# bibymaths/phoskintime

Measured on AMD Instinct MI355X. Metric: ODE-solve replicas/sec (32-state distributive, 14 tp), higher is better.
Workload: dtype f64

## Files before the change

phoskintime_amd/csrc/pk_dist_fast.hpp:

```cpp
#pragma once
#include "pk_dist_rows.hpp"
#include "pk_env.hpp"

namespace pk {

template <int G, int RPL>
__device__ __forceinline__ double site_sum(const double (&s)[RPL], int lane) { return gsum<G>(tree_sum(s), lane); }

enum { PK_DM_NONE = 0, PK_DM_SUM = 1, PK_DM_FULL = 2 };
__host__ __device__ __forceinline__ int dist_metric_class(const SolveArgs& A) {
  return !A.metric ? PK_DM_NONE : (A.metric_id == PK_METRIC_TOTAL_SIGNAL || A.metric_id == PK_METRIC_MEAN_ACTIVITY) ? PK_DM_SUM : PK_DM_FULL;
}
template <bool CLIP, bool NORM, bool FLAT, bool SOL, int MC>
struct DistFixed {
  static constexpr int SLOT_MC = MC;
  static constexpr bool LITERAL = false;
  __host__ __device__ static __forceinline__ bool clip(const SolveArgs&) { return CLIP; }
  __host__ __device__ static __forceinline__ bool normalize(const SolveArgs&) { return NORM; }
  __host__ __device__ static __forceinline__ bool flat(const SolveArgs&) { return FLAT; }
  __host__ __device__ static __forceinline__ bool sol(const SolveArgs&) { return SOL; }
  __host__ __device__ static __forceinline__ int mclass(const SolveArgs&) { return MC; }
  static bool matches(const SolveArgs& A) {
    return (A.clip != 0) == CLIP && (A.normalize != 0) == NORM && (A.flat != nullptr) == FLAT && (A.sol != nullptr) == SOL && dist_metric_class(A) == MC;
  }
};
struct DistAny {
  static constexpr int SLOT_MC = PK_DM_FULL;
  static constexpr bool LITERAL = true;
  __host__ __device__ static __forceinline__ bool clip(const SolveArgs& A) { return A.clip != 0; }
  __host__ __device__ static __forceinline__ bool normalize(const SolveArgs& A) { return A.normalize != 0; }
  __host__ __device__ static __forceinline__ bool flat(const SolveArgs& A) { return A.flat != nullptr; }
  __host__ __device__ static __forceinline__ bool sol(const SolveArgs& A) { return A.sol != nullptr; }
  __host__ __device__ static __forceinline__ int mclass(const SolveArgs& A) { return dist_metric_class(A); }
  static bool matches(const SolveArgs&) { return true; }
};
using DistSolSum = DistFixed<true, false, false, true, PK_DM_SUM>;
using DistSolOnly = DistFixed<true, false, false, true, PK_DM_NONE>;
using DistFlatOnly = DistFixed<true, false, true, false, PK_DM_NONE>;

template <int RPL, int MC, bool RES = false> constexpr int dist_fast_slots() {
  return MC == PK_DM_FULL ? 3 * RPL + (RES ? 4 : 6) : MC == PK_DM_SUM ? 2 * RPL + 1 : 2 * RPL;
}

template <int RPL, bool PARK, int NT> struct Parked;
template <int RPL, int NT> struct Parked<RPL, false, NT> {
  double v[3 * RPL + 6];
  __device__ __forceinline__ explicit Parked(double*) {}
  template <int K> __device__ __forceinline__ double get() const { return v[K]; }
  template <int K> __device__ __forceinline__ void set(double x) { v[K] = x; }
  __device__ __forceinline__ void fence() {}
};
template <int RPL, int NT> struct Parked<RPL, true, NT> {
  typedef __attribute__((address_space(3))) double lds_double;
  lds_double* base;
  __device__ __forceinline__ explicit Parked(double* lds) : base((lds_double*)lds + threadIdx.x) {}
  template <int K> __device__ __forceinline__ double get() const { return base[K * NT]; }
  template <int K> __device__ __forceinline__ void set(double x) { base[K * NT] = x; }
  __device__ __forceinline__ void fence() { asm volatile("" : "+v"(base)); }
};
template <int RPL, bool PARK, int NT = 256, class CFG = DistAny, bool RES = false>
constexpr size_t dist_fast_lds_bytes() { return PARK ? (size_t)(dist_fast_slots<RPL, CFG::SLOT_MC, RES>() + RPL) * NT * sizeof(double) : 0; }

constexpr int PK_DSCHED_K2 = 5, PK_DSCHED_K1 = 9;
constexpr int PK_HWREG_HW_ID = 4 | (31 << 11), PK_HWREG_HW_ID_WAVE = 4 | (3 << 11), PK_HWREG_XCC_ID = 20 | (31 << 11);

template <bool PACE> struct DistPace {
  __device__ __forceinline__ void enter(const SolveArgs&) {}
  __device__ __forceinline__ void step(int) const {}
};
template <> struct DistPace<true> {
  bool paced = false;
  __device__ __forceinline__ void enter(const SolveArgs& A) {
    const int sched = A.sched;
    if (sched != PK_DSCHED_OFF) {
      bool leader = false;
      if ((int)gridDim.x > A.R1) {
        if (sched & PK_DSCHED_LEAD_SLOT) leader = (int)blockIdx.x < A.R1 && __builtin_amdgcn_s_getreg(PK_HWREG_HW_ID_WAVE) == 0;
        if (sched & PK_DSCHED_LEAD_BLOCK) leader = leader || (int)blockIdx.x < A.R1 / 3;
      }
      if (leader) __builtin_amdgcn_s_setprio(3);
      paced = !leader && (sched & PK_DSCHED_LEVEL) != 0;
    }
  }
  __device__ __forceinline__ void step(const int k) const {
    if (paced) {
      if (__builtin_amdgcn_ballot_w64(k < PK_DSCHED_K2) != 0) __builtin_amdgcn_s_setprio(2);
      else if (__builtin_amdgcn_ballot_w64(k < PK_DSCHED_K1) != 0) __builtin_amdgcn_s_setprio(1);
      else __builtin_amdgcn_s_setprio(0);
    }
  }
};

struct DistTraceRec {
  unsigned long long t_entry, t_exit;
  unsigned block, hw_id, xcc_id, iters;
};
struct DistTraceBuf { DistTraceRec* rec; long long capacity; };
template <int TRACE> struct DistTrace;

template <int TRACE> struct DistWaveTrace {
  int witer = 0;
  __device__ __forceinline__ void enter() {
    const unsigned long long t0 = __builtin_amdgcn_s_memrealtime();
    const DistTraceBuf tb = DistTrace<TRACE>::get();
    if (threadIdx.x == 0 && tb.rec && (long long)blockIdx.x < tb.capacity) {
      DistTraceRec* r = tb.rec + blockIdx.x;
      r->t_entry = t0; r->t_exit = 0; r->block = blockIdx.x; r->iters = 0;
      r->hw_id = __builtin_amdgcn_s_getreg(PK_HWREG_HW_ID); r->xcc_id = __builtin_amdgcn_s_getreg(PK_HWREG_XCC_ID);
    }
  }
  __device__ __forceinline__ void step() { ++witer; }
  __device__ __forceinline__ void exit() const {
    int it = witer;
    for (int o = 32; o > 0; o >>= 1) { const int v = __shfl_xor(it, o); it = v > it ? v : it; }
    const DistTraceBuf tb = DistTrace<TRACE>::get();
    if (threadIdx.x == 0 && tb.rec && (long long)blockIdx.x < tb.capacity) {
      DistTraceRec* r = tb.rec + blockIdx.x;
      r->iters = (unsigned)it; r->t_exit = __builtin_amdgcn_s_memrealtime();
    }
  }
};
template <> struct DistWaveTrace<0> {
  __device__ __forceinline__ void enter() {}
  __device__ __forceinline__ void step() {}
  __device__ __forceinline__ void exit() const {}
};

template <int METHOD, int RPL, bool PARK, bool RES> constexpr bool dist_scaled() {
  return PARK && ResolventTab<METHOD>::DIFFERENCE && (RES ? (RPL == 6 || RPL == 8) : (RPL >= 5 && RPL <= 7));
}
constexpr double PK_DIST_SCALE_MIN = 0x1p-600;

template <int G, int RPL, int METHOD, bool PARK = false, int MINB = (PARK ? 2 : 1), int NT = 256, class CFG = DistAny, bool RES = false, int TRACE = 0>
__global__ __launch_bounds__(NT, MINB) void dist_fast_kernel(const SolveArgs A) {
  using Tab = ResolventTab<METHOD>;
  using Vec = Stg<RPL, RES>;
  constexpr bool SCL = dist_scaled<METHOD, RPL, PARK, RES>();
  constexpr int J0 = RES ? 1 : 0;
  static_assert(!SCL || RPL - J0 >= 2, "the scaled rows' dot product runs on two chains");
  static_assert(!TRACE || NT == 64, "the trace holds one record per workgroup: one wave each");
  DistWaveTrace<TRACE> trace;
  trace.enter();
  DistPace<PARK && NT == 64 && METHOD == PK_METHOD_LRP12> pace;
  pace.enter(A);
  extern __shared__ __align__(16) double park_lds[];
  Parked<RPL, PARK, NT> pk(park_lds);
  static_assert(dist_fast_lds_bytes<RPL, PARK, 64, CFG, RES>() * 4 * MINB <= 160 * 1024, "parked slots exceed the CU's LDS at this occupancy");
  constexpr int MCS = CFG::SLOT_MC;
  constexpr int NSL = dist_fast_slots<RPL, MCS, RES>(), FB = 3 * RPL + (RES ? 0 : 2);
  constexpr int K_SR = 0, K_DG = RPL, K_PS = 2 * RPL, K_PR = 3 * RPL, K_PP = 3 * RPL + 1, K_M1 = (MCS == PK_DM_FULL ? FB : 2 * RPL),
                K_M2 = FB + 1, K_MD = FB + 2, K_SH = FB + 3, K_Y = NSL;
  constexpr int RPB = NT / G;
  const int lane = lane_id();
  const int l = threadIdx.x & (G - 1);
  const long long rep = (long long)blockIdx.x * RPB + (threadIdx.x / G);
  if (rep >= A.B) return;
  const int n = A.n_sites, S = A.S, T = A.T;
  const int mclass = CFG::mclass(A);
  const double* __restrict__ th = A.theta + rep * A.P;

  const double cA = th[0], cB = th[1], cC = th[2];
  const bool isR = RES && l == 0, isP = RES && l == 1;
  const double w0 = isR ? cC : 1.0, k3 = isR ? cA : 0.0;
  double lsum = 0.0;
  static_for<RPL>([&](auto jc) {
    constexpr int j = decltype(jc)::value;
    const int i = l + G * j - (RES ? 2 : 0);
    const bool ok = i >= 0 && i < n;
    const double sr = ok ? th[4 + i] : 0.0;
    double dg = ok ? 1.0 + th[4 + n + i] : 1.0;
    if constexpr (RES && j == 0) dg = isR ? cB : isP ? -cC : dg;
    pk.template set<K_SR + j>(sr);
    pk.template set<K_DG + j>(dg);
    lsum += sr;
  });
  const double Dsum = th[3] + gsum<G>(lsum, lane);
  auto sites_only = [&](const auto& s) {
    double v[RPL];
#pragma unroll
    for (int j = 0; j < RPL; ++j) v[j] = s[j];
    v[0] = (isR || isP) ? 0.0 : v[0];
    return gsum<G>(tree_sum(v), lane);
  };

  const double* y0p = A.y0 + (A.y0_batched ? rep * S : 0);
  Vec y;
  if constexpr (!RES) { y.R() = y0p[0]; y.P() = y0p[1]; }
#pragma unroll
  for (int j = 0; j < RPL; ++j) {
    const int i = l + G * j;
    if constexpr (RES) y.s[j] = (i < S) ? y0p[i] : 0.0;
    else y.s[j] = (i < n) ? y0p[2 + i] : 0.0;
  }
  if constexpr (PARK) static_for<RPL>([&](auto jc) { constexpr int j = decltype(jc)::value; pk.template set<K_Y + j>(y.s[j]); });

  static_for<NSL - 2 * RPL>([&](auto kc) { pk.template set<K_PS + decltype(kc)::value>(0.0); });
  const int T5 = T > 5 ? T - 5 : 0;
  double* srow = CFG::sol(A) ? A.sol + rep * T * S + (RES ? 0 : 2) + l : nullptr;
  auto emit = [&](const int k, const Vec& v, auto nf) {
    constexpr bool nan_fill = decltype(nf)::value;
    double* fl = CFG::flat(A) ? A.flat + rep * A.F : nullptr;
    bool clip_now = CFG::clip(A);
    if constexpr (!CFG::LITERAL && !nan_fill) if (clip_now) clip_now = __builtin_amdgcn_ballot_w64(sign_or(v) < 0) != 0;
    auto val = [&](double x, int state) {
      if (nan_fill) return __builtin_nan("");
      double r = (CFG::LITERAL && CFG::clip(A)) ? ((x < 0.0) ? 0.0 : x) : x;
      if (CFG::normalize(A)) r *= 1.0 / y0p[state];
      return r;
    };
    Vec c = v;
    if constexpr (!CFG::LITERAL && !nan_fill) if (clip_now) {
      asm volatile("" : "+v"(c.s[Vec::tree_row(0)]));
      clip_rows(c);
    }
    double vR = 0.0, vP = 0.0;
    if constexpr (!RES) {
      vR = val(c.R(), 0); vP = val(c.P(), 1);
      if (l == 0) {
        if (CFG::sol(A)) { srow[-2] = vR; srow[-1] = vP; }
        if (CFG::flat(A)) { if (k >= 5) fl[k - 5] = vR; fl[T5 + k] = vP; }
      }
    }
    const bool masked = CFG::LITERAL || CFG::normalize(A);
    double vs[RPL];
    double loc = (!RES && l == 0) ? vR + vP : 0.0;
#pragma unroll
    for (int j = 0; j < RPL; ++j) {
      const int i = l + G * j;
      if constexpr (RES) {
        vs[j] = (i < S || !masked) ? val(c.s[j], i) : 0.0;
        if (i < S) {
          if (CFG::sol(A)) srow[G * j] = vs[j];
          if (CFG::flat(A)) if (j > 0 || i > 0 || k >= 5) fl[T5 + (i - 1) * T + k] = vs[j];
        }
      } else {
        vs[j] = (i < n || !masked) ? val(c.s[j], 2 + i) : 0.0;
        if (i < n) {
          if (CFG::sol(A)) srow[G * j] = vs[j];
          if (CFG::flat(A)) fl[T5 + T + i * T + k] = vs[j];
        }
      }
      loc += vs[j];
    }
    if (CFG::sol(A)) srow += S;
    if (mclass != PK_DM_NONE) {
      pk.template set<K_M1>(pk.template get<K_M1>() + loc);
      if constexpr (MCS == PK_DM_FULL) if (mclass == PK_DM_FULL) {
        double m2 = pk.template get<K_M2>(), mdyn = pk.template get<K_MD>(), shift = pk.template get<K_SH>();
        double prevR = 0.0, prevP = 0.0;
        if constexpr (!RES) { prevR = pk.template get<K_PR>(); prevP = pk.template get<K_PP>(); }
        if (k == 0) {
          shift = gsum<G>(loc, lane) / (2 + n);
          pk.template set<K_SH>(shift);
          prevR = vR; prevP = vP;
          static_for<RPL>([&](auto jc) { constexpr int j = decltype(jc)::value; pk.template set<K_PS + j>(vs[j]); });
        }
        static_for<RPL>([&](auto jc) {
          constexpr int j = decltype(jc)::value;
          const int i = l + G * j;
          const double xs = (i < (RES ? S : n)) ? vs[j] - shift : 0.0;
          m2 = __builtin_fma(xs, xs, m2);
          const double d = vs[j] - pk.template get<K_PS + j>();
          mdyn = __builtin_fma(d, d, mdyn);
          pk.template set<K_PS + j>(vs[j]);
        });
        if constexpr (!RES) {
          if (l == 0) {
            const double a = vR - shift, b = vP - shift;
            m2 = __builtin_fma(a, a, m2); m2 = __builtin_fma(b, b, m2);
            const double dR = vR - prevR, dP = vP - prevP;
            mdyn = __builtin_fma(dR, dR, mdyn); mdyn = __builtin_fma(dP, dP, mdyn);
          }
          pk.template set<K_PR>(vR); pk.template set<K_PP>(vP);
        }
        pk.template set<K_M2>(m2); pk.template set<K_MD>(mdyn);
      }
    }
  };
  auto finish = [&](const int status, const int acc, const int rej) {
    if (mclass != PK_DM_NONE) {
      const double L = 2.0 * T + (double)T * n;
      const double tot = gsum<G>(pk.template get<K_M1>(), lane);
      double m = tot;
      if (A.metric_id == PK_METRIC_MEAN_ACTIVITY) m = tot / L;
      if constexpr (MCS == PK_DM_FULL) if (mclass == PK_DM_FULL) {
        const double m2 = pk.template get<K_M2>(), mdyn = pk.template get<K_MD>(), shift = pk.template get<K_SH>();
        switch (A.metric_id) {
          case PK_METRIC_VARIANCE: { const double q = gsum<G>(m2, lane); const double ms = tot / L - shift; m = q / L - ms * ms; } break;
          case PK_METRIC_DYNAMICS: m = gsum<G>(mdyn, lane); break;
          default: { const double q = gsum<G>(m2, lane); m = sqrt(fmax(q + 2.0 * shift * tot - L * shift * shift, 0.0)); } break;
        }
      }
      if (l == 0) A.metric[rep] = m;
    }
    if (l == 0) {
      if (A.status) A.status[rep] = status;
      if (A.n_steps) { A.n_steps[2 * rep] = acc; A.n_steps[2 * rep + 1] = rej; }
    }
  };

  emit(0, y, std::false_type{});
  int status = PK_ST_OK, nacc = 0;
  if (T < 2) { trace.exit(); finish(status, 0, 0); return; }

  const double rtol = A.rtol, atol = A.atol;
  const DistNorm<G, RPL, RES> norm{rtol, atol, lane};
  auto rhs_of = [&](const Vec& Y, const double sg) {
    Vec f;
    if constexpr (RES) {
      const double Rb = bcast<G, 0>(Y.s[0]), Pb = bcast<G, 1>(Y.s[0]);
      static_for<RPL>([&](auto jc) {
        constexpr int j = decltype(jc)::value;
        const double sr = pk.template get<K_SR + j>(), dg = pk.template get<K_DG + j>();
        if constexpr (j == 0) f.s[0] = __builtin_fma(isP ? -Dsum : sr, Pb, __builtin_fma(-dg, isP ? Rb : Y.s[0], isP ? sg : k3));
        else f.s[j] = __builtin_fma(sr, Pb, -dg * Y.s[j]);
      });
    } else {
      f.R() = __builtin_fma(-cB, Y.R(), cA);
      f.P() = __builtin_fma(cC, Y.R(), __builtin_fma(-Dsum, Y.P(), sg));
      static_for<RPL>([&](auto jc) {
        constexpr int j = decltype(jc)::value;
        f.s[j] = __builtin_fma(pk.template get<K_SR + j>(), Y.P(), -pk.template get<K_DG + j>() * Y.s[j]);
      });
    }
    return f;
  };

  double tc = A.t[0];
  int k = 1;
  double te = A.t[1];
  double h;
  {
    double sg0;
    if constexpr (RES) sg0 = sites_only(y.s);
    else {
      double v[RPL];
#pragma unroll
      for (int j = 0; j < RPL; ++j) v[j] = y.s[j];
      sg0 = site_sum<G>(v, lane);
    }
    const Vec f0 = rhs_of(y, sg0);
    const double d0 = norm.group_max(y, y, y), d1 = norm.group_max(f0, y, y);
    h = step_h0(d0, d1, A.h0);
  }
  double is[RPL];
  if constexpr (SCL) static_for<RPL>([&](auto jc) {
    constexpr int j = decltype(jc)::value;
    if constexpr (j >= J0) {
      const double sr = pk.template get<K_SR + j>();
      const double s = !(fabs(sr) < PK_DIST_SCALE_MIN) ? sr : (sr == 0.0 && y.s[j] == 0.0) ? 0.0 : PK_DIST_SCALE_MIN;
      pk.template set<K_SR + j>(s);
      is[j] = s != 0.0 ? 1.0 / s : 0.0;
    }
  });

  double winv[RPL], cw[RPL], omw[RPL], g[RPL], ic[RPL], winvR, omwR, Cl, sinv, Scw, qq, qs, ws0;
  auto factor = [&](const double q) {
    qq = q;
    constexpr int X = RES ? 0 : 1;
    constexpr int NP = RPL + X, M0 = NP <= 5 ? NP : (NP + 1) / 2, M1 = NP - M0;
    double piv[NP];
    if constexpr (!RES) piv[0] = __builtin_fma(q, cB, 1.0);
    static_for<RPL>([&](auto jc) {
      constexpr int j = decltype(jc)::value;
      piv[X + j] = __builtin_fma(q, pk.template get<K_DG + j>(), 1.0);
    });
    if constexpr (RES) piv[0] = isP ? q : piv[0];
    {
      double a[M0], inv[M0];
#pragma unroll
      for (int i = 0; i < M0; ++i) a[i] = piv[i];
      chain_rcp<M0>(a, inv);
      if constexpr (!RES) winvR = inv[0];
#pragma unroll
      for (int i = X; i < M0; ++i) winv[i - X] = inv[i];
    }
    if constexpr (M1 > 0) {
      double a[M1], inv[M1];
#pragma unroll
      for (int i = 0; i < M1; ++i) a[i] = piv[M0 + i];
      chain_rcp<M1>(a, inv);
#pragma unroll
      for (int i = 0; i < M1; ++i) winv[M0 - X + i] = inv[i];
    }
    static_for<RPL>([&](auto jc) {
      constexpr int j = decltype(jc)::value;
      if constexpr (SCL) {
        cw[j] = winv[j] * pk.template get<K_SR + j>();
        omw[j] = (q * winv[j]) * pk.template get<K_DG + j>();
        if constexpr (j >= J0) {
          g[j] = winv[j] * cw[j];
          ic[j] = piv[X + j] * is[j];
        }
      } else if constexpr (Tab::DIFFERENCE) {
        const double qw = q * winv[j];
        cw[j] = qw * pk.template get<K_SR + j>();
        omw[j] = qw * pk.template get<K_DG + j>();
      } else cw[j] = q * pk.template get<K_SR + j>() * winv[j];
    });
    if constexpr (!Tab::DIFFERENCE) Scw = gsum<G>(tree_sum(cw), lane);
    else if constexpr (SCL) {
      if constexpr (!RES) omwR = q * winvR * cB;
      Scw = q * gsum<G>(tree_sum(cw), lane);
    } else if constexpr (!RES) {
      omwR = q * winvR * cB;
      Cl = tree_sum(cw);
      Scw = gsum<G>(Cl, lane);
    } else if constexpr (RPL > 1) {
      double rest[RPL - 1];
#pragma unroll
      for (int j = 1; j < RPL; ++j) rest[j - 1] = cw[j];
      Cl = tree_sum(rest);
      Scw = gsum<G>(Cl + cw[0], lane);
    } else {
      Cl = 0.0;
      Scw = gsum<G>(cw[0], lane);
    }
    sinv = fast_rcp(__builtin_fma(q, Dsum - Scw, 1.0));
    if constexpr (RES) {
      qs = q * sinv;
      if constexpr (SCL) qs *= q;
      ws0 = winv[0] * w0;
      if constexpr (SCL) cw[0] = isP ? winv[0] : cw[0]; else cw[0] = isP ? 1.0 : cw[0];
      winv[0] = isP ? 0.0 : winv[0];
      if constexpr (Tab::DIFFERENCE) omw[0] = isP ? 1.0 : omw[0];
    }
  };
  double lam = 0.0;
  auto gdot = [&](const Vec& v) {
    if constexpr (SCL) {
      constexpr int H = (RPL + J0) / 2;
      double a, b = g[H] * v.s[H];
      if constexpr (RES) a = v.s[0] * ws0; else a = g[0] * v.s[0];
#pragma unroll
      for (int j = 1; j < H; ++j) a = __builtin_fma(g[j], v.s[j], a);
#pragma unroll
      for (int j = H + 1; j < RPL; ++j) b = __builtin_fma(g[j], v.s[j], b);
      return a + b;
    } else return 0.0;
  };
  auto xq_of = [&](const Vec& v, double& xR, double& xP) {
    if constexpr (RES) return gsum<G>(gdot(v), lane) * qs;
    else {
      xR = v.R() * winvR;
      xP = __builtin_fma(qq, __builtin_fma(cC, xR, gsum<G>(gdot(v), lane)), v.P()) * sinv;
      return qq * xP;
    }
  };
  auto solve = [&](const Vec& r, auto first) {
    Vec u;
    double xR = 0.0;
    if constexpr (SCL) {
      double xP = 0.0;
      const double xq = xq_of(r, xR, xP);
      if constexpr (RES) u.s[0] = __builtin_fma(cw[0], xq, r.s[0] * winv[0]);
      else { u.R() = xR; u.P() = xP; }
#pragma unroll
      for (int j = J0; j < RPL; ++j) {
        if constexpr (decltype(first)::value) u.s[j] = __builtin_fma(-omw[j], r.s[j], xq);
        else u.s[j] = __builtin_fma(-omw[j], r.s[j], r.s[j] + xq);
      }
      return u;
    }
    if constexpr (!RES) xR = r.R() * winvR;
    double t[RPL];
#pragma unroll
    for (int j = 0; j < RPL; ++j) t[j] = r.s[j] * winv[j];
    if constexpr (RES) {
      double in, tsum = 0.0;
      if constexpr (RPL > 1) {
        double rest[RPL - 1];
#pragma unroll
        for (int j = 1; j < RPL; ++j) rest[j - 1] = t[j];
        tsum = tree_sum(rest);
        in = __builtin_fma(r.s[0], ws0, tsum);
      } else in = r.s[0] * ws0;
      const double xP = gsum<G>(in, lane) * qs;
      if constexpr (Tab::DIFFERENCE && RPL > 1) lam = __builtin_fma(xP, Cl, tsum);
#pragma unroll
      for (int j = 0; j < RPL; ++j) u.s[j] = __builtin_fma(cw[j], xP, t[j]);
    } else {
      const double tsum = tree_sum(t);
      const double St = gsum<G>(tsum, lane);
      const double xP = __builtin_fma(qq, __builtin_fma(cC, xR, St), r.P()) * sinv;
      if constexpr (Tab::DIFFERENCE) lam = __builtin_fma(xP, Cl, tsum);
#pragma unroll
      for (int j = 0; j < RPL; ++j) u.s[j] = __builtin_fma(cw[j], xP, t[j]);
      u.R() = xR; u.P() = xP;
    }
    return u;
  };
  auto diff = [&](Vec& v) {
    if constexpr (SCL) {
      double xR = 0.0, xP = 0.0;
      const double xq = xq_of(v, xR, xP);
      if constexpr (RES) v.s[0] = __builtin_fma(-cw[0], xq, omw[0] * v.s[0]);
      else { v.R() *= omwR; v.P() -= xP; }
#pragma unroll
      for (int j = J0; j < RPL; ++j) v.s[j] = __builtin_fma(omw[j], v.s[j], -xq);
      return;
    }
    double p[RPL];
#pragma unroll
    for (int j = 0; j < RPL; ++j) p[j] = omw[j] * v.s[j];
    if constexpr (RES) {
      double in, psum = 0.0;
      if constexpr (RPL > 1) {
        double rest[RPL - 1];
#pragma unroll
        for (int j = 1; j < RPL; ++j) rest[j - 1] = p[j];
        psum = tree_sum(rest);
        in = __builtin_fma(v.s[0], ws0, lam - psum);
      } else in = v.s[0] * ws0;
      const double xP = gsum<G>(in, lane) * qs;
#pragma unroll
      for (int j = 0; j < RPL; ++j) v.s[j] = __builtin_fma(-cw[j], xP, p[j]);
      if constexpr (RPL > 1) lam = __builtin_fma(-xP, Cl, psum);
    } else {
      const double psum = tree_sum(p);
      const double xR = v.R() * winvR;
      const double St = gsum<G>(lam - psum, lane);
      const double xP = __builtin_fma(qq, __builtin_fma(cC, xR, St), v.P()) * sinv;
#pragma unroll
      for (int j = 0; j < RPL; ++j) v.s[j] = __builtin_fma(-cw[j], xP, p[j]);
      lam = __builtin_fma(-xP, Cl, psum);
      v.R() *= omwR; v.P() -= xP;
    }
  };

  bool after_reject = false;
  auto state_bad = [&]() {
    double rows[RPL];
#pragma unroll
    for (int j = 0; j < RPL; ++j) rows[j] = y.s[j];
    if constexpr (PARK) {
      pk.fence();
      static_for<RPL>([&](auto jc) { constexpr int j = decltype(jc)::value; rows[j] = pk.template get<K_Y + j>(); });
    }
    bool b;
    if constexpr (RES) b = ((isR || isP) && nonfinite(rows[0])) || nonfinite(sites_only(rows));
    else b = (nonfinite(y.R())) || (nonfinite(y.P())) || (nonfinite(site_sum<G>(rows, lane)));
    return gmax<G>(b ? 1.0 : 0.0, lane);
  };
  auto coef_bad = [&]() {
    if constexpr (RES) {
      long long r2 = rep;
      asm volatile("" : "+v"(r2));
      const double* t2 = A.theta + r2 * A.P;
      return (nonfinite(t2[0])) || (nonfinite(t2[1])) || (nonfinite(t2[2]));
    } else return (nonfinite(cA)) || (nonfinite(cB)) || (nonfinite(cC));
  };
  int nsec = 0;
  __builtin_amdgcn_s_waitcnt(0x0F70);
  while (true) {
    bool nonfin = false;
    while (true) {
      trace.step();
      pace.step(k);
      const double tnx = A.t[k + 1 < T ? k + 1 : T - 1];
      const bool over = (CFG::LITERAL ? nacc + nsec : nsec) >= A.max_steps;
      const bool last = (tc + 1.0001 * h >= te);
      const double hs = last ? te - tc : ((tc + 2.0 * h > te) ? 0.5 * (te - tc) : h);
      if (over || !(hs > 1e-14 * max_abs_k(tc, 1e-3))) { status |= over ? PK_ST_MAXSTEPS : PK_ST_HMIN; break; }
      if constexpr (PARK) {
        pk.fence();
        static_for<RPL>([&](auto jc) { constexpr int j = decltype(jc)::value; y.s[j] = pk.template get<K_Y + j>(); });
      }
      factor(Tab::GAM * hs);

      Vec z;
      {
        Vec r = y;
        if constexpr (RES) r.s[0] = __builtin_fma(qq, k3, y.s[0]); else r.R() = __builtin_fma(qq, cA, y.R());
        if constexpr (SCL) {
#pragma unroll
          for (int j = J0; j < RPL; ++j) r.s[j] = y.s[j] * ic[j];
          z = solve(r, std::true_type{});
#pragma unroll
          for (int j = 0; j < Vec::NR; ++j) if (j < J0 || j >= RPL) z.s[j] -= y.s[j];
        } else {
          z = solve(r, std::false_type{});
          trk_axpy(z, -1.0, y);
        }
      }
      Vec yn = y;
      if constexpr (SCL) {
#pragma unroll
        for (int j = J0; j < RPL; ++j) yn.s[j] = 0.0;
      }
      trk_axpy(yn, Tab::B[0] / Tab::GAM, z);
      double err;
      if constexpr (Tab::DIFFERENCE) {
        z = solve(z, std::false_type{});
        trk_axpy(yn, Tab::BN[0] / Tab::GAM, z);
        static_for<Tab::NS - 2>([&](auto mc) {
          constexpr int m = 1 + decltype(mc)::value;
          diff(z);
          trk_axpy(yn, Tab::BN[m] / Tab::GAM, z);
        });
        if constexpr (SCL) {
          pk.fence();
          static_for<RPL - J0>([&](auto jc) { constexpr int j = J0 + decltype(jc)::value; y.s[j] = pk.template get<K_Y + j>(); });
#pragma unroll
          for (int j = J0; j < RPL; ++j) {
            yn.s[j] = __builtin_fma(cw[j], yn.s[j], y.s[j]);
            z.s[j] *= cw[j];
          }
        }
        constexpr double e1 = (Tab::E[1] < 0.0 ? -Tab::E[1] : Tab::E[1]) / Tab::GAM;
        if constexpr (CFG::LITERAL) err = e1 * norm.group_max(z, y, yn); else err = e1 * norm.err_norm(z, y, yn);
      } else {
        Vec u6;
        static_for<Tab::NS - 1>([&](auto kc) {
          constexpr int kk = 1 + decltype(kc)::value;
          constexpr double bk = Tab::B[kk] / Tab::GAM, ek = Tab::E[kk] / Tab::GAM;
          z = solve(z, std::false_type{});
          trk_axpy(yn, bk, z);
          if constexpr (kk == 1) u6 = trk_scale(ek, z); else trk_axpy(u6, ek, z);
        });
        if constexpr (CFG::LITERAL) err = norm.group_max(u6, y, yn); else err = norm.err_norm(u6, y, yn);
      }
      const bool acc = (err <= 1.0);
      if constexpr (PARK) {
        if (acc) {
          static_for<RPL>([&](auto jc) { constexpr int j = decltype(jc)::value; pk.template set<K_Y + j>(yn.s[j]); });
          if constexpr (!CFG::LITERAL) tc += hs;
        }
#pragma unroll
        for (int j = 0; j < RPL; ++j) y.s[j] = yn.s[j];
        #pragma unroll
        for (int x = 0; x < Vec::X; ++x) y.s[RPL + x] = acc ? yn.s[RPL + x] : y.s[RPL + x];
      } else {
        if (acc) {
          y = yn;
          if constexpr (!CFG::LITERAL) tc += hs;
        }
      }
      if constexpr (CFG::LITERAL) {
        if (err != err || err > 1e300) {
          ++nsec; after_reject = true; h = 0.1 * hs;
          if (state_bad() != 0.0 || coef_bad() || (nonfinite(Dsum)) || (nonfinite(Scw))) {
            status |= PK_ST_NONFINITE; break;
          }
          continue;
        }
      } else {
        ++nsec;
        if (__builtin_expect(err != err || err > 1e300, 0)) { after_reject = true; h = 0.1 * hs; nonfin = true; break; }
      }
      const float e32 = (float)min_raw_k(max_raw_k(err, 1e-30), 1e30);
      const double finv = step_growth((double)__builtin_amdgcn_exp2f(__builtin_amdgcn_logf(e32) * (float)(-1.0 / Tab::Q)));
      double hnew = hs * finv;
      const bool land = acc && last;
      if constexpr (CFG::LITERAL) { nacc += acc ? 1 : 0; nsec += acc ? 0 : 1; }
      else nacc += (int)acc;
      if (acc && after_reject) hnew = min_raw(hnew, hs);
      after_reject = !acc;
      if constexpr (CFG::LITERAL) tc = land ? te : (acc ? tc + hs : tc);
      h = (land && hs < h) ? max_raw(hnew, h) : hnew;
      if (land) {
        if constexpr (!CFG::LITERAL) tc = te;
        te = tnx;
        asm volatile("" : "+v"(te));
        emit(k, y, std::false_type{});
        ++k;
      }
      if (k >= T) break;
    }
    if (CFG::LITERAL || !nonfin) break;
    if (state_bad() != 0.0 || coef_bad() || (nonfinite(Dsum)) || (nonfinite(Scw))) {
      status |= PK_ST_NONFINITE; break;
    }
  }
  const int nrej = CFG::LITERAL ? nsec : nsec - nacc;
  if (status != PK_ST_OK)
    for (; k < T; ++k) emit(k, y, std::true_type{});
  trace.exit();
  finish(status, nacc, nrej);
}

}
```

Baseline: 269.0 million.

## Fold stage-one scaling into solve and make P-slot selects arithmetic

For scaled configurations, the inverse scale is premultiplied by the diagonal once at setup. The first-stage solve then uses winv directly instead of building ic[] and rescaling the right-hand side every step. For selected resolvent configurations, the per-step isP selects on the P slot become FMA/multiply arithmetic with precomputed 0/1 masks, with the diagonal slot overwritten at setup. The scaled dot product is also collapsed from two FMA chains into a single chain. This trims per-step ALU work and selects, but the single chain lengthens dependency latency and the reordered arithmetic may change rounding.

Result: faster. 279.6 million, median of 6 (+3.9%).

```diff
diff --git a/phoskintime_amd/csrc/pk_dist_fast.hpp b/phoskintime_amd/csrc/pk_dist_fast.hpp
--- a/phoskintime_amd/csrc/pk_dist_fast.hpp
+++ b/phoskintime_amd/csrc/pk_dist_fast.hpp
@@ -130,6 +130,13 @@
   return PARK && ResolventTab<METHOD>::DIFFERENCE && (RES ? (RPL == 6 || RPL == 8) : (RPL >= 5 && RPL <= 7));
 }
 constexpr double PK_DIST_SCALE_MIN = 0x1p-600;
+template <int METHOD, int RPL, bool PARK, bool RES> constexpr bool dist_stage1_state() {
+  return dist_scaled<METHOD, RPL, PARK, RES>() && (RES ? RPL == 8 : RPL != 5);
+}
+template <int RPL, class CFG> constexpr bool dist_pslot_arith() {
+  constexpr bool any = std::is_same<CFG, DistAny>::value, flat = std::is_same<CFG, DistFlatOnly>::value;
+  return !(RPL == 1 && any) && !(RPL == 2 && flat) && !(RPL == 5 && !any && !flat) && !(RPL == 6 && flat);
+}
 
 template <int G, int RPL, int METHOD, bool PARK = false, int MINB = (PARK ? 2 : 1), int NT = 256, class CFG = DistAny, bool RES = false, int TRACE = 0>
 __global__ __launch_bounds__(NT, MINB) void dist_fast_kernel(const SolveArgs A) {
@@ -137,7 +144,8 @@
   using Vec = Stg<RPL, RES>;
   constexpr bool SCL = dist_scaled<METHOD, RPL, PARK, RES>();
   constexpr int J0 = RES ? 1 : 0;
-  static_assert(!SCL || RPL - J0 >= 2, "the scaled rows' dot product runs on two chains");
+  constexpr bool S1 = dist_stage1_state<METHOD, RPL, PARK, RES>();
+  constexpr bool PAR = RES && dist_pslot_arith<RPL, CFG>();
   static_assert(!TRACE || NT == 64, "the trace holds one record per workgroup: one wave each");
   DistWaveTrace<TRACE> trace;
   trace.enter();
@@ -351,8 +359,14 @@
       const double s = !(fabs(sr) < PK_DIST_SCALE_MIN) ? sr : (sr == 0.0 && y.s[j] == 0.0) ? 0.0 : PK_DIST_SCALE_MIN;
       pk.template set<K_SR + j>(s);
       is[j] = s != 0.0 ? 1.0 / s : 0.0;
+      if constexpr (S1) is[j] *= pk.template get<K_DG + j>();
     }
   });
+  double selP = isP ? 1.0 : 0.0, notP = isP ? 0.0 : 1.0;
+  if constexpr (PAR) {
+    if (isP) pk.template set<K_DG + 0>(1.0);
+    asm volatile("" : "+v"(selP), "+v"(notP));
+  }
 
   double winv[RPL], cw[RPL], omw[RPL], g[RPL], ic[RPL], winvR, omwR, Cl, sinv, Scw, qq, qs, ws0;
   auto factor = [&](const double q) {
@@ -363,9 +377,10 @@
     if constexpr (!RES) piv[0] = __builtin_fma(q, cB, 1.0);
     static_for<RPL>([&](auto jc) {
       constexpr int j = decltype(jc)::value;
-      piv[X + j] = __builtin_fma(q, pk.template get<K_DG + j>(), 1.0);
+      if constexpr (PAR && j == 0) piv[0] = __builtin_fma(q, pk.template get<K_DG + 0>(), notP);
+      else piv[X + j] = __builtin_fma(q, pk.template get<K_DG + j>(), 1.0);
     });
-    if constexpr (RES) piv[0] = isP ? q : piv[0];
+    if constexpr (RES && !PAR) piv[0] = isP ? q : piv[0];
     {
       double a[M0], inv[M0];
 #pragma unroll
@@ -390,7 +405,7 @@
         omw[j] = (q * winv[j]) * pk.template get<K_DG + j>();
         if constexpr (j >= J0) {
           g[j] = winv[j] * cw[j];
-          ic[j] = piv[X + j] * is[j];
+          if constexpr (!S1) ic[j] = piv[X + j] * is[j];
         }
       } else if constexpr (Tab::DIFFERENCE) {
         const double qw = q * winv[j];
@@ -421,29 +436,32 @@
       qs = q * sinv;
       if constexpr (SCL) qs *= q;
       ws0 = winv[0] * w0;
-      if constexpr (SCL) cw[0] = isP ? winv[0] : cw[0]; else cw[0] = isP ? 1.0 : cw[0];
-      winv[0] = isP ? 0.0 : winv[0];
-      if constexpr (Tab::DIFFERENCE) omw[0] = isP ? 1.0 : omw[0];
+      if constexpr (PAR) {
+        if constexpr (SCL) cw[0] = __builtin_fma(winv[0], selP, cw[0]); else cw[0] += selP;
+        winv[0] *= notP;
+        if constexpr (Tab::DIFFERENCE) omw[0] = __builtin_fma(omw[0], notP, selP);
+      } else {
+        if constexpr (SCL) cw[0] = isP ? winv[0] : cw[0]; else cw[0] = isP ? 1.0 : cw[0];
+        winv[0] = isP ? 0.0 : winv[0];
+        if constexpr (Tab::DIFFERENCE) omw[0] = isP ? 1.0 : omw[0];
+      }
     }
   };
   double lam = 0.0;
-  auto gdot = [&](const Vec& v) {
+  auto gdot = [&](const Vec& v, const double (&c)[RPL]) {
     if constexpr (SCL) {
-      constexpr int H = (RPL + J0) / 2;
-      double a, b = g[H] * v.s[H];
-      if constexpr (RES) a = v.s[0] * ws0; else a = g[0] * v.s[0];
-#pragma unroll
-      for (int j = 1; j < H; ++j) a = __builtin_fma(g[j], v.s[j], a);
-#pragma unroll
-      for (int j = H + 1; j < RPL; ++j) b = __builtin_fma(g[j], v.s[j], b);
-      return a + b;
+      double a;
+      if constexpr (RES) a = v.s[0] * ws0; else a = c[0] * v.s[0];
+#pragma unroll
+      for (int j = 1; j < RPL; ++j) a = __builtin_fma(c[j], v.s[j], a);
+      return a;
     } else return 0.0;
   };
-  auto xq_of = [&](const Vec& v, double& xR, double& xP) {
-    if constexpr (RES) return gsum<G>(gdot(v), lane) * qs;
+  auto xq_of = [&](const Vec& v, const double (&c)[RPL], double& xR, double& xP) {
+    if constexpr (RES) return gsum<G>(gdot(v, c), lane) * qs;
     else {
       xR = v.R() * winvR;
-      xP = __builtin_fma(qq, __builtin_fma(cC, xR, gsum<G>(gdot(v), lane)), v.P()) * sinv;
+      xP = __builtin_fma(qq, __builtin_fma(cC, xR, gsum<G>(gdot(v, c), lane)), v.P()) * sinv;
       return qq * xP;
     }
   };
@@ -452,12 +470,14 @@
     double xR = 0.0;
     if constexpr (SCL) {
       double xP = 0.0;
-      const double xq = xq_of(r, xR, xP);
+      constexpr bool state = S1 && decltype(first)::value;
+      const double xq = state ? xq_of(r, winv, xR, xP) : xq_of(r, g, xR, xP);
       if constexpr (RES) u.s[0] = __builtin_fma(cw[0], xq, r.s[0] * winv[0]);
       else { u.R() = xR; u.P() = xP; }
 #pragma unroll
       for (int j = J0; j < RPL; ++j) {
-        if constexpr (decltype(first)::value) u.s[j] = __builtin_fma(-omw[j], r.s[j], xq);
+        if constexpr (state) u.s[j] = __builtin_fma(-qq, is[j] * r.s[j], xq);
+        else if constexpr (decltype(first)::value) u.s[j] = __builtin_fma(-omw[j], r.s[j], xq);
         else u.s[j] = __builtin_fma(-omw[j], r.s[j], r.s[j] + xq);
       }
       return u;
@@ -493,7 +513,7 @@
   auto diff = [&](Vec& v) {
     if constexpr (SCL) {
       double xR = 0.0, xP = 0.0;
-      const double xq = xq_of(v, xR, xP);
+      const double xq = xq_of(v, g, xR, xP);
       if constexpr (RES) v.s[0] = __builtin_fma(-cw[0], xq, omw[0] * v.s[0]);
       else { v.R() *= omwR; v.P() -= xP; }
 #pragma unroll
@@ -573,8 +593,10 @@
         Vec r = y;
         if constexpr (RES) r.s[0] = __builtin_fma(qq, k3, y.s[0]); else r.R() = __builtin_fma(qq, cA, y.R());
         if constexpr (SCL) {
-#pragma unroll
-          for (int j = J0; j < RPL; ++j) r.s[j] = y.s[j] * ic[j];
+          if constexpr (!S1) {
+#pragma unroll
+            for (int j = J0; j < RPL; ++j) r.s[j] = y.s[j] * ic[j];
+          }
           z = solve(r, std::true_type{});
 #pragma unroll
           for (int j = 0; j < Vec::NR; ++j) if (j < J0 || j >= RPL) z.s[j] -= y.s[j];
```
